# liuzuxin/FSRL

Hardware: NVIDIA H100
Metric: env-steps/sec (collect+update) SafetyCarCircle-v0 PPO-Lag (higher is better)
Workload: dtype f32

## Files before the change

### fsrl_b200/csrc/ppo_persist.cu

```cuda
#include "ppo_persist.cuh"
#include "arena.cuh"
#include "ppo_loss.cuh"
#include "wgmma.cuh"
#include <cstdlib>
#include <cmath>
#include <vector>

namespace fsrl {
namespace pp {

using namespace wg;

constexpr int WQ = 2;
constexpr int NEPI = 128 * WQ;
constexpr int TPB = NEPI + 32;
constexpr int C1 = 16 / WQ;
constexpr int C2 = 32 / WQ;
constexpr int RB = 64;
constexpr int MB = 256;
constexpr int KC = 32, NCH = 256 / KC;
constexpr int SLOT_BYTES = 32768, NSLOT = 4;
constexpr int A_CHUNK = 64 * KC * 4;
constexpr int ACC_LD = 68;
constexpr int OUTP = 8;
constexpr int H_ = 256;
constexpr int IMG = 65536;
enum { I_H1A_HI, I_H1A_LO, I_H1T_HI, I_H1T_LO, I_DZA_HI, I_DZA_LO, I_DZT_HI, I_DZT_LO, I_W2A_HI, I_W2A_LO, I_W2B_HI, I_W2B_LO, N_IMG };
constexpr int DB2P_OFF = N_IMG * IMG;
constexpr int DW3P_OFF = DB2P_OFF + 4 * H_;
constexpr int DB3P_OFF = DW3P_OFF + 4 * H_ * OUTP;
constexpr int DW1P_OFF = DB3P_OFF + 4 * 16;
constexpr int MAXD = 40;
constexpr int NET_WS = DW1P_OFF + 4 * WQ * (MAXD + 1) * H_;
constexpr int SUMSQ_FLOATS = 128;
constexpr int FLAG_LINE = 32;
constexpr int F_A = 0, F_C = 1, F_D1 = 2, F_PER_NET = 3;
constexpr int NSMAX = (MAXD + 1) * 32 + 32 + 32 * OUTP + 16;
constexpr int TILE_PK = (64 * 64 / NEPI + 2) / 3;
constexpr int TILE_FLOATS = TILE_PK * NEPI * 4;
constexpr int SLICE_PK = (NSMAX + 2) / 3;
constexpr int XG_PER_NET = 16 * TILE_FLOATS + 8 * SLICE_PK * 4;
constexpr int MAX_MB = 16384;
constexpr long long WAIT_CYCLES = 6000000000LL;

struct Args {
    fsrl_ppo_update_t u;
    int n_mb, slot0;
    long long adam_t0;
    float* ws;
    unsigned* flags;
    int* err;
    const float* adam_tab;
    long long* dbg;
    int dbg_step;
    unsigned dp_seq;
    int dp_direct;
};
constexpr int DBG_N = 48;
#define STAMP(i) do { if (P.dbg && t == P.dbg_step) P.dbg[(size_t)blockIdx.x * DBG_N + (i)] = clock64(); } while (0)

struct AdamS { float w1, b2, w2, rbc2s, eps, neg_step; };
__device__ __forceinline__ float adam_one(float p, float g, float& m, float& v, const AdamS& a) {
    m = m + a.w1 * (g - m);
    v = v * a.b2 + (a.w2 * g) * g;
    const float sq = v > 0.f ? v * rsqrtf(v) : 0.f;
    const float denom = fmaf(sq, a.rbc2s, a.eps);
    return p + __fdividef(a.neg_step * m, denom);
}

__device__ __forceinline__ void fail(int* err, int code) {
    *reinterpret_cast<volatile int*>(err) = code;
    __threadfence_system();
    asm volatile("trap;");
}
__device__ __forceinline__ uint32_t pk_hash(float x, float y, float z) {
    const uint32_t a = __float_as_uint(x), b = __float_as_uint(y), c = __float_as_uint(z);
    return a ^ __funnelshift_l(b, b, 11) ^ __funnelshift_l(c, c, 22);
}
__device__ __forceinline__ bool pk_ok(const float4& v, uint32_t tag) { return (__float_as_uint(v.w) ^ pk_hash(v.x, v.y, v.z)) == tag; }
__device__ __forceinline__ void st_packet(float* p, float x, float y, float z, uint32_t tag) {
    asm volatile("st.relaxed.sys.global.v4.f32 [%0], {%1,%2,%3,%4};" ::"l"(p), "f"(x), "f"(y), "f"(z), "f"(__uint_as_float(tag ^ pk_hash(x, y, z))) : "memory");
}
__device__ __forceinline__ float4 ld_packet(const float* p) {
    float4 v;
    asm volatile("ld.relaxed.sys.global.v4.f32 {%0,%1,%2,%3}, [%4];" : "=f"(v.x), "=f"(v.y), "=f"(v.z), "=f"(v.w) : "l"(p) : "memory");
    return v;
}

__device__ __noinline__ float3 dp_gather(const float* src, long long stride, int me, int world, uint32_t tag,
                                        float ox, float oy, float oz, int* err, int code) {
    const long long t0w = clock64();
    float ax = 0.f, ay = 0.f, az = 0.f;
    for (int r0 = 0; r0 < world; r0 += 4) {
        float4 v[4];
        bool ok;
        do {
            ok = true;
#pragma unroll
            for (int k = 0; k < 4; ++k)
                if (r0 + k < world && r0 + k != me) v[k] = ld_packet(src + (size_t)(r0 + k) * stride);
#pragma unroll
            for (int k = 0; k < 4; ++k)
                if (r0 + k < world && r0 + k != me) ok = ok && pk_ok(v[k], tag);
            if (!ok && clock64() - t0w > 4 * WAIT_CYCLES) fail(err, code);
        } while (!ok);
#pragma unroll
        for (int k = 0; k < 4; ++k) {
            if (r0 + k >= world) continue;
            if (r0 + k == me) { ax += ox; ay += oy; az += oz; }
            else { ax += v[k].x; ay += v[k].y; az += v[k].z; }
        }
    }
    return make_float3(ax, ay, az);
}
__device__ __noinline__ void dp_push_all(const float* const* xg, size_t off, int me, int world, float x, float y, float z, uint32_t tag) {
    for (int r = 0; r < world; ++r)
        if (r != me) st_packet(const_cast<float*>(xg[r]) + off, x, y, z, tag);
}

__device__ __forceinline__ uint32_t mapa_u32(uint32_t local_saddr, uint32_t rank) {
    uint32_t r;
    asm volatile("mapa.shared::cluster.u32 %0, %1, %2;" : "=r"(r) : "r"(local_saddr), "r"(rank));
    return r;
}
__device__ __forceinline__ void st_cluster4(uint32_t raddr, float4 v) {
    asm volatile("st.shared::cluster.v4.f32 [%0], {%1,%2,%3,%4};" ::"r"(raddr), "f"(v.x), "f"(v.y), "f"(v.z), "f"(v.w) : "memory");
}
__device__ __forceinline__ void st_async4(uint32_t raddr, float4 v, uint32_t rbar) {
    asm volatile("st.async.weak.shared::cluster.mbarrier::complete_tx::bytes.v4.f32 [%0], {%1,%2,%3,%4}, [%5];"
                 ::"r"(raddr), "f"(v.x), "f"(v.y), "f"(v.z), "f"(v.w), "r"(rbar) : "memory");
}
__device__ __forceinline__ bool mbar_wait_cluster(uint64_t* bar, uint32_t parity, long long timeout_cycles) {
    const long long t0 = clock64();
    while (true) {
        uint32_t ok;
        asm volatile(
            "{\n\t.reg .pred p;\n\t"
            "mbarrier.try_wait.parity.acquire.cluster.shared::cta.b64 p, [%1], %2;\n\t"
            "selp.u32 %0, 1, 0, p;\n\t}"
            : "=r"(ok) : "r"(smem_u32(bar)), "r"(parity) : "memory");
        if (ok) return true;
        if (clock64() - t0 > timeout_cycles) return false;
    }
}
__device__ __forceinline__ void cluster_sync_all() {
    asm volatile("barrier.cluster.arrive.release.aligned;\n\tbarrier.cluster.wait.acquire.aligned;" ::: "memory");
}

__device__ __forceinline__ bool elect_one() {
    uint32_t pred = 0;
    asm volatile(
        "{\n\t.reg .b32 rx;\n\t.reg .pred px;\n\t"
        "elect.sync rx|px, 0xffffffff;\n\t"
        "selp.u32 %0, 1, 0, px;\n\t}"
        : "=r"(pred));
    return pred != 0;
}
__device__ __forceinline__ void epi_bar() { asm volatile("bar.sync 1, %0;" ::"n"(NEPI) : "memory"); }
__device__ __forceinline__ void prefetch_l2(const void* p) { asm volatile("prefetch.global.L2 [%0];" ::"l"(p)); }

template <int NC>
__device__ __forceinline__ void acc_ld(const float* accs, int row, int col, float (&v)[NC]) {
#pragma unroll
    for (int q = 0; q < NC / 4; ++q) {
        const float4 x = *reinterpret_cast<const float4*>(accs + row * ACC_LD + col + 4 * q);
        v[4 * q] = x.x; v[4 * q + 1] = x.y; v[4 * q + 2] = x.z; v[4 * q + 3] = x.w;
    }
}
template <int NC>
__device__ __forceinline__ void acc_st(float* accs, int row, int col, const float (&v)[NC]) {
#pragma unroll
    for (int q = 0; q < NC / 4; ++q)
        *reinterpret_cast<float4*>(accs + row * ACC_LD + col + 4 * q) = make_float4(v[4 * q], v[4 * q + 1], v[4 * q + 2], v[4 * q + 3]);
}

template <int N>
__device__ __forceinline__ void gemm_phase(const unsigned char* ring, unsigned& qq, uint64_t* bar_full, uint32_t empty_r,
                                           float (&dm)[N / 2], float (&dc)[N / 2], int* err, int code, int lane) {
#pragma unroll
    for (int e = 0; e < N / 2; ++e) dm[e] = dc[e] = 0.f;
    const uint32_t ring_a = smem_u32(ring);
    constexpr uint32_t b_lbo = 16 * N, b_chunk = N * KC * 4;
    for (int j = 0; j < NCH; ++j, ++qq) {
        const int s = qq % NSLOT;
        if (!mbar_wait(&bar_full[s], (qq / NSLOT) & 1, WAIT_CYCLES)) fail(err, code);
        __syncwarp();
        wgmma_fence();
        const uint32_t base = ring_a + (uint32_t)s * SLOT_BYTES;
        const uint64_t ah0 = smem_desc(base, 1024, 128), al0 = smem_desc(base + A_CHUNK, 1024, 128);
        const uint64_t bh0 = smem_desc(base + 2 * A_CHUNK, b_lbo, 128), bl0 = smem_desc(base + 2 * A_CHUNK + b_chunk, b_lbo, 128);
#pragma unroll
        for (int ks = 0; ks < KC / 8; ++ks) {
            const uint64_t ah = ah0 + ks * (2048 / 16), al = al0 + ks * (2048 / 16);
            const uint64_t bh = bh0 + ks * (2 * b_lbo / 16), bl = bl0 + ks * (2 * b_lbo / 16);
            if constexpr (N == 32) {
                mma_m64n32k8_tf32(dc, al, bh);
                mma_m64n32k8_tf32(dc, ah, bl);
                mma_m64n32k8_tf32(dm, ah, bh);
            } else {
                mma_m64n64k8_tf32(dc, al, bh);
                mma_m64n64k8_tf32(dc, ah, bl);
                mma_m64n64k8_tf32(dm, ah, bh);
            }
        }
        wgmma_commit();
        if (j > 0) {
            wgmma_wait<1>();
            __syncwarp();
            if (lane < 8) mbar_arrive_cluster(empty_r + 8 * ((qq - 1) % NSLOT));
        }
    }
    wgmma_wait<0>();
    reg_fence(dm); reg_fence(dc);
    __syncwarp();
// ... 99 lines not shown
    float g[C2];
    acc_ld<C2>(accs, trow, cb2, g);
    const float inv_world = 1.0f / (float)d.world;
    const float* loc = d.xg[d.me];
#pragma unroll
    for (int q = 0; q < TILE_PK; ++q) {
        if (dp_owner(et, q, d.world) != d.me) continue;
        const float3 s3 = dp_gather(loc + off + (size_t)q * NEPI * 4, d.region, d.me, d.world, d.tag, g[3 * q],
                                    3 * q + 1 < C2 ? g[3 * q + 1] : 0.f, 3 * q + 2 < C2 ? g[3 * q + 2] : 0.f, d.err, 41);
        const float ax = s3.x * inv_world, ay = s3.y * inv_world, az = s3.z * inv_world;
        dp_push_all(d.xg, (size_t)FSRL_P2P_MAX_RANKS * d.region + off + (size_t)q * NEPI * 4, d.me, d.world, ax, ay, az, d.tag);
        g[3 * q] = ax;
        if (3 * q + 1 < C2) g[3 * q + 1] = ay;
        if (3 * q + 2 < C2) g[3 * q + 2] = az;
    }
    acc_st<C2>(accs, trow, cb2, g);
}
__device__ __noinline__ float dp_tile_finish(DpCtx d, size_t off, float* accs, int trow, int cb2, int et) {
    float g[C2];
    const long long t0w = clock64();
    if (d.direct) {
        float own[C2];
        acc_ld<C2>(accs, trow, cb2, own);
#pragma unroll
        for (int jq = 0; jq < C2; ++jq) g[jq] = 0.f;
        for (int r = 0; r < d.world; ++r) {
            if (r == d.me) {
#pragma unroll
                for (int jq = 0; jq < C2; ++jq) g[jq] += own[jq];
                continue;
            }
            const float* src = d.xg[d.me] + (size_t)r * d.region + off;
            float4 v[TILE_PK];
            bool ok;
            do {
                ok = true;
#pragma unroll
                for (int q = 0; q < TILE_PK; ++q) v[q] = ld_packet(src + (size_t)q * NEPI * 4);
#pragma unroll
                for (int q = 0; q < TILE_PK; ++q) ok = ok && pk_ok(v[q], d.tag);
                if (!ok && clock64() - t0w > 4 * WAIT_CYCLES) fail(d.err, 42);
            } while (!ok);
#pragma unroll
            for (int q = 0; q < TILE_PK; ++q) {
                g[3 * q] += v[q].x;
                if (3 * q + 1 < C2) g[3 * q + 1] += v[q].y;
                if (3 * q + 2 < C2) g[3 * q + 2] += v[q].z;
            }
        }
        const float inv_world = 1.0f / (float)d.world;
        float sq = 0.f;
#pragma unroll
        for (int jq = 0; jq < C2; ++jq) { g[jq] *= inv_world; sq = fmaf(g[jq], g[jq], sq); }
        acc_st<C2>(accs, trow, cb2, g);
        return sq;
    }
    const float* res = d.xg[d.me] + (size_t)FSRL_P2P_MAX_RANKS * d.region + off;
    acc_ld<C2>(accs, trow, cb2, g);
    float4 v[TILE_PK];
    bool ok;
    do {
        ok = true;
#pragma unroll
        for (int q = 0; q < TILE_PK; ++q)
            if (dp_owner(et, q, d.world) != d.me) v[q] = ld_packet(res + (size_t)q * NEPI * 4);
#pragma unroll
        for (int q = 0; q < TILE_PK; ++q)
            if (dp_owner(et, q, d.world) != d.me) ok = ok && pk_ok(v[q], d.tag);
        if (!ok && clock64() - t0w > 4 * WAIT_CYCLES) fail(d.err, 42);
    } while (!ok);
    float sq = 0.f;
#pragma unroll
    for (int q = 0; q < TILE_PK; ++q) {
        if (dp_owner(et, q, d.world) == d.me) continue;
        g[3 * q] = v[q].x;
        if (3 * q + 1 < C2) g[3 * q + 1] = v[q].y;
        if (3 * q + 2 < C2) g[3 * q + 2] = v[q].z;
    }
#pragma unroll
    for (int jq = 0; jq < C2; ++jq) sq = fmaf(g[jq], g[jq], sq);
    acc_st<C2>(accs, trow, cb2, g);
    return sq;
}
__device__ __noinline__ void dp_slices(DpCtx d, size_t off_s, float* sp_g, int n, int et, bool push) {
    const int n3 = (n + 2) / 3;
    const float inv_world = 1.0f / (float)d.world;
    if (push)
        for (int i = et; i < n3; i += NEPI)
            dp_push_all(d.xg, (size_t)d.me * d.region + off_s + 4 * (size_t)i, d.me, d.world,
                        sp_g[3 * i], 3 * i + 1 < n ? sp_g[3 * i + 1] : 0.f, 3 * i + 2 < n ? sp_g[3 * i + 2] : 0.f, d.tag);
    const float* loc = d.xg[d.me];
    for (int i = et; i < n3; i += NEPI) {
        const float3 s3 = dp_gather(loc + off_s + 4 * (size_t)i, d.region, d.me, d.world, d.tag, sp_g[3 * i],
                                    3 * i + 1 < n ? sp_g[3 * i + 1] : 0.f, 3 * i + 2 < n ? sp_g[3 * i + 2] : 0.f, d.err, 40);
        sp_g[3 * i] = s3.x * inv_world;
        if (3 * i + 1 < n) sp_g[3 * i + 1] = s3.y * inv_world;
        if (3 * i + 2 < n) sp_g[3 * i + 2] = s3.z * inv_world;
    }
}

template <bool DP>
__global__ void __launch_bounds__(TPB, 1) ppo_persist_kernel(const Args P) {
    extern __shared__ __align__(1024) unsigned char smem_raw[];
    __shared__ __align__(8) uint64_t bar_full[NSLOT], bar_empty[NSLOT], bar_b;
    __shared__ float s_red[4][320];
    __shared__ float s_misc[32];
    __shared__ AdamS s_adam;
    __shared__ const float* s_xg[2][FSRL_P2P_MAX_RANKS];
    const fsrl_ppo_update_t& u = P.u;
    const int tid = threadIdx.x, warp = tid >> 5, lane = tid & 31;
    const int net = blockIdx.x >> 5, c = blockIdx.x & 31, a = c >> 3, b = c & 7;
    const bool is_g2 = c < 16;
    const int ka = (c & 15) >> 2, q4 = c & 3;
    const int D = u.D, A = u.A, C = u.C, H = H_;
    const int out = (net == 0) ? A : 1;
    const int n_cta = 32 * u.n_nets;
    float* wsn = P.ws + (size_t)net * NET_WS;
    float* sumsq_g = P.ws + (size_t)u.n_nets * NET_WS;
    unsigned* fl_net = P.flags + (size_t)net * F_PER_NET * FLAG_LINE;
    unsigned* fl_d2 = P.flags + (size_t)u.n_nets * F_PER_NET * FLAG_LINE;
    unsigned char* ring = smem_raw;
    float* accs = reinterpret_cast<float*>(smem_raw + NSLOT * SLOT_BYTES);
    float* small = accs + 64 * ACC_LD;
    const SliceMap sm(D);
    float* sp_p = small;
    float* sp_m = small + sm.n;
    float* sp_v = small + 2 * sm.n;
    float* sp_g = small + 3 * sm.n;
    float* land = small + 4 * sm.n;

    if (tid == 0) {
        for (int i = 0; i < NSLOT; ++i) { mbar_init(&bar_full[i], 1); mbar_init(&bar_empty[i], 4 * 8); }
        mbar_init(&bar_b, 1);
        fence_mbar_init();
    }
    __syncthreads();
    if (DP && threadIdx.x < 2 * FSRL_P2P_MAX_RANKS) s_xg[threadIdx.x / FSRL_P2P_MAX_RANKS][threadIdx.x % FSRL_P2P_MAX_RANKS] = P.u.p2p_xg[threadIdx.x / FSRL_P2P_MAX_RANKS][threadIdx.x % FSRL_P2P_MAX_RANKS];
    if (DP) __syncthreads();
    cluster_sync_all();

    const long long pbase = u.net_off[net];
    const ArenaLayout L = arena_layout(D, H, out, 0);
    const long long o_w1 = pbase + L.w1, o_b1 = pbase + L.b1, o_w2 = pbase + L.w2, o_b2 = pbase + L.b2,
                    o_w3 = pbase + L.w3, o_b3 = pbase + L.b3, o_ls = pbase + L.extra;

    if (warp == NEPI / 32) {
        if (elect_one()) {
            unsigned qq = 0;
            for (int t = 0; t < P.n_mb; ++t) {
                if (!flag_wait_ge<true>(fl_net + F_A * FLAG_LINE, 32u * (t + 1), WAIT_CYCLES)) fail(P.err, 10);
                STAMP(12);
                fence_proxy_async();
#pragma unroll 1
                for (int j = 0; j < NCH; ++j, ++qq) {
                    const int s = qq % NSLOT;
                    if (!mbar_wait(&bar_empty[s], ((qq / NSLOT) & 1) ^ 1, WAIT_CYCLES)) fail(P.err, 11);
                    unsigned char* dst = ring + (size_t)s * SLOT_BYTES;
                    mbar_expect_tx(&bar_full[s], 3 * A_CHUNK);
                    const size_t ao = (size_t)a * 16384 + (size_t)j * 64 * KC, bo = (size_t)b * 8192 + (size_t)j * 32 * KC;
                    copy_operand(dst, wsn + (size_t)I_H1A_HI * IMG + ao, A_CHUNK, &bar_full[s], 8, b, 0xff);
                    copy_operand(dst + 2 * A_CHUNK, wsn + (size_t)I_W2A_HI * IMG + bo, A_CHUNK / 2, &bar_full[s], 1, 0, 0);
                }
                STAMP(13);
                if (!flag_wait_ge<true>(fl_net + F_C * FLAG_LINE, 32u * (t + 1), WAIT_CYCLES)) fail(P.err, 12);
                STAMP(14);
                fence_proxy_async();
                const int ia = is_g2 ? I_W2B_HI : I_DZT_HI, ib = is_g2 ? I_DZA_HI : I_H1T_HI;
                const int blk_a = is_g2 ? ka : q4, blk_b = is_g2 ? q4 : ka;
                const uint16_t m4 = (uint16_t)(0xfu << (b & 4)), m2 = (uint16_t)(0x11u << (b & 3));
#pragma unroll 1
                for (int j = 0; j < NCH; ++j, ++qq) {
                    const int s = qq % NSLOT;
                    if (!mbar_wait(&bar_empty[s], ((qq / NSLOT) & 1) ^ 1, WAIT_CYCLES)) fail(P.err, 13);
                    unsigned char* dst = ring + (size_t)s * SLOT_BYTES;
                    mbar_expect_tx(&bar_full[s], 4 * A_CHUNK);
                    const size_t ao = (size_t)blk_a * 16384 + (size_t)j * 64 * KC, bo = (size_t)blk_b * 16384 + (size_t)j * 64 * KC;
                    copy_operand(dst, wsn + (size_t)ia * IMG + ao, A_CHUNK, &bar_full[s], is_g2 ? 4 : 2, is_g2 ? b & 3 : b >> 2, is_g2 ? m4 : m2);
                    copy_operand(dst + 2 * A_CHUNK, wsn + (size_t)ib * IMG + bo, A_CHUNK, &bar_full[s], is_g2 ? 2 : 4, is_g2 ? b >> 2 : b & 3, is_g2 ? m2 : m4);
                }
            }
        }
    } else {
        const int et = tid;
        const int sp = warp & 3;
        const int wq = warp >> 2;
        const int r16 = lane & 15, half = lane >> 4;
        const int trow = 16 * sp + r16;
        const int cb1 = 16 * half + C1 * wq;
        const int cb2 = 32 * half + C2 * wq;
        unsigned qq = 0;
        const uint32_t empty_r = mapa_u32(smem_u32(bar_empty), lane < 8 ? lane : 0);
        float w2p[C2], w2m[C2], w2v[C2];
        const int world = DP ? u.world : 1;
        auto dp_ctx = [&](int t_) {
            DpCtx d;
            const unsigned long long id = (unsigned long long)(P.adam_t0 + t_ + 1);
            d.xg = s_xg[(int)(id & 1ULL)];
            d.region = (long long)u.n_nets * XG_PER_NET;
            d.me = u.p2p_rank; d.world = world;
            d.tag = (P.dp_seq << 16) | (uint32_t)((t_ + 1) & 0xffff);
            d.err = P.err;
            d.direct = P.dp_direct;
            return d;
        };

        for (int i = et; i < sm.n; i += NEPI) {
            long long src = -1;
            if (i < sm.b2) { const int d = i / 32, kk = i % 32; src = (d < D) ? o_w1 + (long long)d * H + 32 * b + kk : o_b1 + 32 * b + kk; }
            else if (i < sm.w3) src = o_b2 + 32 * b + (i - sm.b2);
            else if (i < sm.b3) { const int oo = (i - sm.w3) / OUTP, jj = (i - sm.w3) % OUTP; if (jj < out) src = o_w3 + (long long)(32 * b + oo) * out + jj; }
            else { const int jj = i - sm.b3; if (jj < out) src = o_b3 + jj; else if (net == 0 && jj >= 8 && jj < 8 + A) src = o_ls + (jj - 8); }
            sp_p[i] = src >= 0 ? u.theta[src] : 0.f;
            sp_m[i] = src >= 0 ? u.adam_m[src] : 0.f;
            sp_v[i] = src >= 0 ? u.adam_v[src] : 0.f;
            sp_g[i] = 0.f;
        }
// ... 209 lines not shown
#pragma unroll
                for (int q = 0; q < C1 / 4; ++q) {
#pragma unroll
                    for (int e = 0; e < 4; ++e) tf32_split(dz[4 * q + e], hi[4 * q + e], lo[4 * q + e]);
                    const size_t plane = (size_t)(8 * b + (cb1 >> 2) + q) * 256;
                    *reinterpret_cast<float4*>(a_hi + plane) = make_float4(hi[4 * q], hi[4 * q + 1], hi[4 * q + 2], hi[4 * q + 3]);
                    *reinterpret_cast<float4*>(a_hi + IMG + plane) = make_float4(lo[4 * q], lo[4 * q + 1], lo[4 * q + 2], lo[4 * q + 3]);
                }
                store_transposed<C1, 32>(scratch, hi, lo, trow, cb1, et, wsn + (size_t)I_DZT_HI * IMG + (size_t)(b >> 1) * 16384, 64 * a, 32 * (b & 1));
            }
            if (et == 0) STAMP(27);
            {
                float* row = &s_red[sp][0];
#pragma unroll
                for (int j = 0; j < C1; ++j) {
                    const float sdz = half_sum(dz[j]);
                    if (r16 == 0) row[cb1 + j] = sdz;
                }
#pragma unroll
                for (int jj = 0; jj < OUTP; ++jj) {
                    if (jj < nfeed) {
#pragma unroll
                        for (int j = 0; j < C1; ++j) {
                            const float sv = half_sum(h2[j] * dd[jj]);
                            if (r16 == 0) row[32 + 32 * jj + cb1 + j] = sv;
                        }
                    }
                }
                if (b == 0 && wq == 0) {
#pragma unroll
                    for (int j = 0; j < 16; ++j) {
                        const float sv = half_sum(dd[j]);
                        if (lane == 0) row[288 + j] = sv;
                    }
                    const float sa = half_sum(st_a), sb = half_sum(st_b), sc = half_sum(st_c), sdv = half_sum(st_d);
                    if (lane == 0) { row[304] = sa; row[305] = sb; row[306] = sc; row[307] = sdv; }
                }
            }
            epi_bar();
            if (et == 0) STAMP(28);
            for (int i = et; i < 32 + 32 * nfeed; i += NEPI) {
                const float tot = ((s_red[0][i] + s_red[1][i]) + s_red[2][i]) + s_red[3][i];
                if (i < 32) wsn[DB2P_OFF + a * H + 32 * b + i] = tot;
                else wsn[DW3P_OFF + ((size_t)a * H + 32 * b + ((i - 32) & 31)) * OUTP + ((i - 32) >> 5)] = tot;
            }
            if (b == 0) {
                if (et < 20) {
                    const int i = 288 + et;
                    const float tot = ((s_red[0][i] + s_red[1][i]) + s_red[2][i]) + s_red[3][i];
                    if (et < 16) wsn[DB3P_OFF + a * 16 + et] = tot;
                    else {
                        float* stat = u.stats + (size_t)slot * FSRL_PPO_STATS;
                        if (net == 0) { if (et == 16) atomicAdd(stat + ST_ACTOR_REW, tot); if (et == 17) atomicAdd(stat + ST_ACTOR_SAFETY, tot); if (et == 18) atomicAdd(stat + ST_KL, tot); }
                        else if (et == 19) atomicAdd(stat + ST_VF0 + (net - 1), tot);
                    }
                }
                if (net == 0 && a == 0 && et == 20) u.stats[(size_t)slot * FSRL_PPO_STATS + ST_ENTROPY] = ppo_entropy(sp_p + sm.b3 + 8, A);
            }
            fence_proxy_async_smem();
            epi_bar();
            if (et == 0) { STAMP(5); flag_add_release(fl_net + F_C * FLAG_LINE); }

            unsigned mbits = 0;
            if (is_g2) {
                const int k = 64 * ka + trow;
                const float* msk = wsn + (size_t)I_H1A_HI * IMG + (size_t)q4 * 16384 + (size_t)(k >> 2) * 256 + (k & 3);
                float mreg[C2];
#pragma unroll
                for (int jq = 0; jq < C2; ++jq) mreg[jq] = __ldcg(msk + (size_t)(cb2 + jq) * 4);
                float xr[(64 * MAXD + NEPI - 1) / NEPI];
                const int nx = (64 * D + NEPI - 1) / NEPI;
                const float* xb = u.obs + (row0 + 64 * q4) * D;
#pragma unroll
                for (int q = 0; q < (64 * MAXD + NEPI - 1) / NEPI; ++q)
                    xr[q] = (q < nx && et + q * NEPI < 64 * D) ? __ldg(xb + et + q * NEPI) : 0.f;
#pragma unroll
                for (int jq = 0; jq < C2; ++jq) mbits |= (mreg[jq] > 0.f ? 1u : 0u) << jq;
#pragma unroll
                for (int q = 0; q < (64 * MAXD + NEPI - 1) / NEPI; ++q) {
                    const int e = et + q * NEPI;
                    if (q < nx && e < 64 * D) { const int r = e / D; land[e + (r >> 5)] = xr[q]; }
                }
            }
            {
                float dm[32], dc[32];
                if (wq == 0) gemm_phase<64>(ring, qq, bar_full, empty_r, dm, dc, P.err, 32, lane);
                else qq += NCH;
                stage_acc<64>(accs, dm, dc, wq, sp, lane);
            }
            if (et == 0) STAMP(6);
            float sq = 0.f;
            if (is_g2) {
                float v[C2];
                acc_ld<C2>(accs, trow, cb2, v);
                const int k = 64 * ka + trow;
#pragma unroll
                for (int jq = 0; jq < C2; ++jq) v[jq] = ((mbits >> jq) & 1u) ? v[jq] : 0.f;
                epi_bar();
                if (et == 0) STAMP(22);
                const float* xh = land + (size_t)cb2 * D + half;
                float* dst = wsn + DW1P_OFF + (size_t)(WQ * q4 + wq) * (MAXD + 1) * H + k;
                for (int d = 0; d < D; ++d) {
                    float sacc = 0.f;
#pragma unroll
                    for (int jq = 0; jq < C2; ++jq) sacc = fmaf(xh[jq * D + d], v[jq], sacc);
                    sacc += __shfl_xor_sync(0xffffffffu, sacc, 16);
                    if (half == 0) dst[(size_t)d * H] = sacc;
                }
                float sb1 = 0.f;
#pragma unroll
                for (int jq = 0; jq < C2; ++jq) sb1 += v[jq];
                sb1 += __shfl_xor_sync(0xffffffffu, sb1, 16);
                if (half == 0) dst[(size_t)D * H] = sb1;
                if (et == 0) STAMP(23);
                epi_bar();
                if (et == 0) flag_add_release(fl_net + F_D1 * FLAG_LINE);
            } else {
                float g[C2];
                acc_ld<C2>(accs, trow, cb2, g);
                if (DP) {
                    dp_tile_send(dp_ctx(t), (size_t)(net * 16 + (c - 16)) * TILE_FLOATS + (size_t)et * 4, accs, trow, cb2, et);
                    if (et == 0) STAMP(32);
                } else {
#pragma unroll
                    for (int jq = 0; jq < C2; ++jq) sq = fmaf(g[jq], g[jq], sq);
                }
            }
            auto reduce_slices = [&](int lo, int hi) {
                for (int i0 = lo + et; i0 < hi; i0 += 4 * NEPI) {
                    float pv[4][4 * WQ];
                    bool real[4];
                    int np[4];
#pragma unroll
                    for (int e = 0; e < 4; ++e) {
                        const int i = i0 + e * NEPI;
                        const float* src = wsn;
                        size_t stride = 0;
                        real[e] = false;
                        np[e] = 4;
                        if (i < hi) {
                            if (i < sm.b2) { src = wsn + DW1P_OFF + (size_t)(i / 32) * H + 32 * b + (i % 32); stride = (size_t)(MAXD + 1) * H; real[e] = true; np[e] = 4 * WQ; }
                            else if (i < sm.w3) { src = wsn + DB2P_OFF + 32 * b + (i - sm.b2); stride = H; real[e] = true; }
                            else if (i < sm.b3) {
                                const int oo = (i - sm.w3) / OUTP, jj = (i - sm.w3) % OUTP;
                                real[e] = jj < out;
                                src = wsn + DW3P_OFF + ((size_t)32 * b + oo) * OUTP + jj; stride = (size_t)H * OUTP;
                            } else {
                                const int jj = i - sm.b3;
                                real[e] = (jj < out) || (net == 0 && jj >= 8 && jj < 8 + A);
                                src = wsn + DB3P_OFF + jj; stride = 16;
                            }
                        }
#pragma unroll
                        for (int q = 0; q < 4 * WQ; ++q) pv[e][q] = (real[e] && q < np[e]) ? __ldcg(src + q * stride) : 0.f;
                    }
#pragma unroll
                    for (int e = 0; e < 4; ++e) {
                        const int i = i0 + e * NEPI;
                        if (i < hi) {
                            float gsum = 0.f;
#pragma unroll
                            for (int q = 0; q < 4 * WQ; ++q) gsum += pv[e][q];
                            sp_g[i] = gsum;
                        }
                    }
                }
            };
            reduce_slices(sm.b2, sm.n);
            if (et == 0) { STAMP(7); if (!flag_wait_ge(fl_net + F_D1 * FLAG_LINE, 16u * (t + 1), WAIT_CYCLES)) fail(P.err, 33); STAMP(8); }
            epi_bar();
            reduce_slices(0, sm.b2);
            if (DP) {
                const DpCtx d = dp_ctx(t);
                const size_t off_t = (size_t)(net * 16 + (c - 16)) * TILE_FLOATS + (size_t)et * 4;
                epi_bar();
                if (!is_g2 && !d.direct) { dp_tile_reduce(d, off_t, accs, trow, cb2, et); if (et == 0) STAMP(33); }
                dp_slices(d, (size_t)u.n_nets * 16 * TILE_FLOATS + (size_t)(net * 8 + b) * SLICE_PK * 4, sp_g, sm.n, et, a == 0);
                __syncwarp();
                if (et == 0) STAMP(38);
                if (!is_g2) { sq += dp_tile_finish(d, off_t, accs, trow, cb2, et); if (et == 0) STAMP(41); }
                epi_bar();
            }
            if (a == 0) {
                for (int i = et; i < sm.n; i += NEPI) {
                    bool real = true;
                    if (i >= sm.w3 && i < sm.b3) real = ((i - sm.w3) % OUTP) < out;
                    else if (i >= sm.b3) { const int jj = i - sm.b3; real = (jj < out) || (net == 0 && jj >= 8 && jj < 8 + A); }
                    if (real && (i < sm.b3 || b == 0)) sq = fmaf(sp_g[i], sp_g[i], sq);
                }
            }
            sq = warp_sum(sq);
            if (lane == 0) s_misc[warp] = sq;
            epi_bar();
            if (et == 0) {
                float tot = 0.f;
#pragma unroll
                for (int w2 = 0; w2 < NEPI / 32; ++w2) tot += s_misc[w2];
                sumsq_g[blockIdx.x] = tot;
                STAMP(9);
                flag_add_release(fl_d2);
                if (!flag_wait_ge(fl_d2, (unsigned)n_cta * (t + 1), WAIT_CYCLES)) fail(P.err, 34);
                STAMP(10);
            }
            epi_bar();
            float nq[4];
#pragma unroll
            for (int q = 0; q < 4; ++q) nq[q] = (lane + 32 * q < n_cta) ? __ldcg(sumsq_g + lane + 32 * q) : 0.f;
            float nsq = ((nq[0] + nq[1]) + nq[2]) + nq[3];
            nsq = warp_sum(nsq);
            float gscale = 1.0f;
            if (u.max_grad_norm > 0.f) gscale = fminf(u.max_grad_norm / (sqrtf(nsq) + 1e-6f), 1.0f);
            if (blockIdx.x == 0 && et == 0) u.stats[(size_t)slot * FSRL_PPO_STATS + ST_GRADNORM] = sqrtf(nsq);
            const AdamS ad = s_adam;
            if (et == 0) STAMP(24);
            for (int i = et; i < sm.n; i += NEPI) {
                float m = sp_m[i], v = sp_v[i];
                sp_p[i] = adam_one(sp_p[i], sp_g[i] * gscale, m, v, ad);
                sp_m[i] = m; sp_v[i] = v;
            }
            if (et == 0) STAMP(25);
            if (!is_g2) {
                float g[C2];
                acc_ld<C2>(accs, trow, cb2, g);
#pragma unroll
                for (int j = 0; j < C2; ++j) w2p[j] = adam_one(w2p[j], g[j] * gscale, w2m[j], w2v[j], ad);
            }
            epi_bar();
            if (et == 0) STAMP(11);
        }

        if (a == 0) {
            for (int i = et; i < sm.n; i += NEPI) {
                long long dst = -1;
                if (i < sm.b2) { const int d = i / 32, kk = i % 32; dst = (d < D) ? o_w1 + (long long)d * H + 32 * b + kk : o_b1 + 32 * b + kk; }
                else if (i < sm.w3) dst = o_b2 + 32 * b + (i - sm.b2);
                else if (i < sm.b3) { const int oo = (i - sm.w3) / OUTP, jj = (i - sm.w3) % OUTP; if (jj < out) dst = o_w3 + (long long)(32 * b + oo) * out + jj; }
                else if (b == 0) { const int jj = i - sm.b3; if (jj < out) dst = o_b3 + jj; else if (net == 0 && jj >= 8 && jj < 8 + A) dst = o_ls + (jj - 8); }
                if (dst >= 0) { u.theta[dst] = sp_p[i]; u.adam_m[dst] = sp_m[i]; u.adam_v[dst] = sp_v[i]; }
            }
        }
        if (!is_g2) {
            const int o = 64 * q4 + trow;
#pragma unroll
            for (int j = 0; j < C2; ++j) {
                const long long idx = o_w2 + (long long)(64 * ka + cb2 + j) * H + o;
                u.theta[idx] = w2p[j]; u.adam_m[idx] = w2m[j]; u.adam_v[idx] = w2v[j];
            }
        }
    }
    __syncthreads();
    cluster_sync_all();
}

static size_t smem_bytes(int D) {
    return (size_t)NSLOT * SLOT_BYTES + sizeof(float) * 64 * ACC_LD + 4 * sizeof(float) * SliceMap(D).n +
           sizeof(float) * 8 * 64 * OUTP;
}

static cudaLaunchConfig_t cluster_launch(int n_nets, size_t smem, cudaStream_t s, cudaLaunchAttribute* at) {
    at->id = cudaLaunchAttributeClusterDimension;
    at->val.clusterDim.x = 8; at->val.clusterDim.y = 1; at->val.clusterDim.z = 1;
    cudaLaunchConfig_t cfg = {};
    cfg.gridDim = dim3(32 * n_nets); cfg.blockDim = dim3(TPB); cfg.dynamicSmemBytes = smem; cfg.stream = s;
    cfg.attrs = at; cfg.numAttrs = 1;
    return cfg;
}

struct Instance {
    void (*kern)(const Args);
    int max_clusters;
};
static const Instance& instance(bool dp) {
    static Instance inst[2] = {};
    Instance& in = inst[dp];
    if (!in.kern) {
        in.kern = dp ? ppo_persist_kernel<true> : ppo_persist_kernel<false>;
        cudaLaunchAttribute at;
        const cudaLaunchConfig_t cfg = cluster_launch(1, smem_bytes(MAXD), nullptr, &at);
        if (cudaFuncSetAttribute(in.kern, cudaFuncAttributeMaxDynamicSharedMemorySize, (int)cfg.dynamicSmemBytes) != cudaSuccess ||
            cudaOccupancyMaxActiveClusters(&in.max_clusters, in.kern, &cfg) != cudaSuccess) {
            cudaGetLastError();
            in.max_clusters = 0;
        }
    }
    return in;
}

}

size_t ppo_persist_ws_floats(int n_nets, int D, int H) {
    (void)D; (void)H;
    return (size_t)n_nets * pp::NET_WS + pp::SUMSQ_FLOATS + (size_t)(n_nets * pp::F_PER_NET + 1) * pp::FLAG_LINE + 32 +
           2 * (size_t)pp::MAX_MB + 2 * (size_t)32 * n_nets * pp::DBG_N;
}

size_t ppo_persist_p2p_floats(int n_nets) { return (size_t)(FSRL_P2P_MAX_RANKS + 1) * n_nets * pp::XG_PER_NET + 64; }

bool ppo_persist_supported(const fsrl_ppo_update_t& u, long long n_total, int batch_size) {
    if (u.H != 256 || batch_size != pp::MB || n_total % pp::MB != 0 || n_total < pp::MB || n_total / pp::MB > pp::MAX_MB) return false;
    if (u.world > 1 && !(u.p2p_on && u.world <= FSRL_P2P_MAX_RANKS && (size_t)u.p2p_stride >= ppo_persist_p2p_floats(u.n_nets))) return false;
    if (u.D < 1 || u.D > pp::MAXD || u.A > 8 || u.n_nets < 1 || u.n_nets > 3) return false;
    if (u.persist_ws == nullptr || (size_t)u.persist_ws_floats < ppo_persist_ws_floats(u.n_nets, u.D, u.H)) return false;
    if (32 * u.n_nets > sm_count()) return false;
    return pp::instance(u.world > 1).max_clusters >= 4 * u.n_nets;
}

int ppo_persist_run(const fsrl_ppo_update_t& ug, int n_mb, int stats_slot0, long long adam_t0, cudaStream_t s) {
    pp::Args a;
    a.u = ug;
    a.n_mb = n_mb; a.slot0 = stats_slot0; a.adam_t0 = adam_t0;
    a.ws = ug.persist_ws;
    const size_t fl_off = (size_t)ug.n_nets * pp::NET_WS + pp::SUMSQ_FLOATS;
    a.flags = reinterpret_cast<unsigned*>(ug.persist_ws + fl_off);
    const size_t n_flag_words = (size_t)(ug.n_nets * pp::F_PER_NET + 1) * pp::FLAG_LINE;
    a.err = reinterpret_cast<int*>(a.flags + n_flag_words);
    FSRL_CUDA(cudaMemsetAsync(a.flags, 0, (n_flag_words + 32) * sizeof(unsigned), s));
    float* tab_dev = reinterpret_cast<float*>(a.err + 32);
    static std::vector<float> tab;
    tab.resize(2 * (size_t)n_mb);
    for (int t = 0; t < n_mb; ++t) {
        const double tt = (double)(adam_t0 + t + 1);
        const double bc1 = 1.0 - pow(ug.beta1, tt), bc2 = 1.0 - pow(ug.beta2, tt);
        tab[2 * t] = (float)(1.0 / sqrt(bc2));
        tab[2 * t + 1] = (float)(-(ug.lr / bc1));
    }
    FSRL_CUDA(cudaMemcpyAsync(tab_dev, tab.data(), tab.size() * sizeof(float), cudaMemcpyHostToDevice, s));
    a.adam_tab = tab_dev;
    static unsigned dp_seq = 0;
    if (ug.world > 1) dp_seq = (dp_seq % 65535u) + 1u;
    a.dp_seq = dp_seq;
    a.dp_direct = ug.world <= 2;
    if (const char* e = getenv("FSRL_PPO_DP_DIRECT")) a.dp_direct = atoi(e) != 0;
    a.dbg = nullptr; a.dbg_step = -1;
    if (const char* e = getenv("FSRL_PPO_PERSIST_DBG")) {
        a.dbg = reinterpret_cast<long long*>(tab_dev + 2 * (size_t)pp::MAX_MB);
        a.dbg_step = atoi(e);
    }
    cudaLaunchAttribute at;
    const cudaLaunchConfig_t cfg = pp::cluster_launch(ug.n_nets, pp::smem_bytes(ug.D), s, &at);
    FSRL_CUDA(cudaLaunchKernelEx(&cfg, pp::instance(ug.world > 1).kern, a));
    ++g_launches;
    return FSRL_OK;
}

}
```

Baseline: 2.611 million.

## Reduce W1 gradient slices through cluster DSMEM with mbarrier signalling

Per-CTA W1 gradient partials now stay in shared memory (the ring buffer) and are summed by designated reducer CTAs, which read them over distributed shared memory after a cluster mbarrier arrive. Before, every CTA wrote them to global workspace and waited on a global flag. The small b2/w3/b3 slice reduction moves earlier, onto the second warpgroup of the reducer CTAs, so it overlaps with the GEMM phase. Only reducer CTAs and g1 CTAs now take part in the global sum-of-squares barrier. The other CTAs read reduced slices back from a global slice buffer, which adds an extra global round trip and tighter coupling to the cluster layout.

```diff
diff --git a/fsrl_b200/csrc/ppo_persist.cu b/fsrl_b200/csrc/ppo_persist.cu
--- a/fsrl_b200/csrc/ppo_persist.cu
+++ b/fsrl_b200/csrc/ppo_persist.cu
@@ -29,13 +29,13 @@
 constexpr int DB2P_OFF = N_IMG * IMG;
 constexpr int DW3P_OFF = DB2P_OFF + 4 * H_;
 constexpr int DB3P_OFF = DW3P_OFF + 4 * H_ * OUTP;
-constexpr int DW1P_OFF = DB3P_OFF + 4 * 16;
 constexpr int MAXD = 40;
-constexpr int NET_WS = DW1P_OFF + 4 * WQ * (MAXD + 1) * H_;
+constexpr int NSMAX = (MAXD + 1) * 32 + 32 + 32 * OUTP + 16;
+constexpr int SLICE_OFF = DB3P_OFF + 4 * 16;
+constexpr int NET_WS = SLICE_OFF + 8 * NSMAX;
 constexpr int SUMSQ_FLOATS = 128;
 constexpr int FLAG_LINE = 32;
-constexpr int F_A = 0, F_C = 1, F_D1 = 2, F_PER_NET = 3;
-constexpr int NSMAX = (MAXD + 1) * 32 + 32 + 32 * OUTP + 16;
+constexpr int F_A = 0, F_C = 1, F_PER_NET = 2;
 constexpr int TILE_PK = (64 * 64 / NEPI + 2) / 3;
 constexpr int TILE_FLOATS = TILE_PK * NEPI * 4;
 constexpr int SLICE_PK = (NSMAX + 2) / 3;
@@ -130,6 +130,14 @@
     asm volatile("st.async.weak.shared::cluster.mbarrier::complete_tx::bytes.v4.f32 [%0], {%1,%2,%3,%4}, [%5];"
                  ::"r"(raddr), "f"(v.x), "f"(v.y), "f"(v.z), "f"(v.w), "r"(rbar) : "memory");
 }
+__device__ __forceinline__ float ld_cluster(uint32_t raddr) {
+    float v;
+    asm volatile("ld.shared::cluster.f32 %0, [%1];" : "=f"(v) : "r"(raddr) : "memory");
+    return v;
+}
+__device__ __forceinline__ void mbar_arrive_release_cluster(uint32_t raddr) {
+    asm volatile("mbarrier.arrive.release.cluster.shared::cluster.b64 _, [%0];" ::"r"(raddr) : "memory");
+}
 __device__ __forceinline__ bool mbar_wait_cluster(uint64_t* bar, uint32_t parity, long long timeout_cycles) {
     const long long t0 = clock64();
     while (true) {
@@ -395,13 +403,12 @@
     acc_st<C2>(accs, trow, cb2, g);
     return sq;
 }
-__device__ __noinline__ void dp_slices(DpCtx d, size_t off_s, float* sp_g, int n, int et, bool push) {
+__device__ __noinline__ void dp_slices(DpCtx d, size_t off_s, float* sp_g, int n, int et) {
     const int n3 = (n + 2) / 3;
     const float inv_world = 1.0f / (float)d.world;
-    if (push)
-        for (int i = et; i < n3; i += NEPI)
-            dp_push_all(d.xg, (size_t)d.me * d.region + off_s + 4 * (size_t)i, d.me, d.world,
-                        sp_g[3 * i], 3 * i + 1 < n ? sp_g[3 * i + 1] : 0.f, 3 * i + 2 < n ? sp_g[3 * i + 2] : 0.f, d.tag);
+    for (int i = et; i < n3; i += NEPI)
+        dp_push_all(d.xg, (size_t)d.me * d.region + off_s + 4 * (size_t)i, d.me, d.world,
+                    sp_g[3 * i], 3 * i + 1 < n ? sp_g[3 * i + 1] : 0.f, 3 * i + 2 < n ? sp_g[3 * i + 2] : 0.f, d.tag);
     const float* loc = d.xg[d.me];
     for (int i = et; i < n3; i += NEPI) {
         const float3 s3 = dp_gather(loc + off_s + 4 * (size_t)i, d.region, d.me, d.world, d.tag, sp_g[3 * i],
@@ -412,10 +419,20 @@
     }
 }
 
+__device__ __forceinline__ bool red_cta() { return ((blockIdx.x >> 3) & 3) == ((blockIdx.x & 7) >> 2); }
+
+__device__ __noinline__ float dp_tail(DpCtx d, size_t off_t, size_t off_s, float* accs, float* sp_g, int n, int trow, int cb2,
+                                      int et, bool tile, bool slice) {
+    if (tile && !d.direct) dp_tile_reduce(d, off_t, accs, trow, cb2, et);
+    if (slice) dp_slices(d, off_s, sp_g, n, et);
+    __syncwarp();
+    return tile ? dp_tile_finish(d, off_t, accs, trow, cb2, et) : 0.f;
+}
+
 template <bool DP>
 __global__ void __launch_bounds__(TPB, 1) ppo_persist_kernel(const Args P) {
     extern __shared__ __align__(1024) unsigned char smem_raw[];
-    __shared__ __align__(8) uint64_t bar_full[NSLOT], bar_empty[NSLOT], bar_b;
+    __shared__ __align__(8) uint64_t bar_full[NSLOT], bar_empty[NSLOT], bar_b, bar_w1;
     __shared__ float s_red[4][320];
     __shared__ float s_misc[32];
     __shared__ AdamS s_adam;
@@ -425,6 +442,7 @@
     const int net = blockIdx.x >> 5, c = blockIdx.x & 31, a = c >> 3, b = c & 7;
     const bool is_g2 = c < 16;
     const int ka = (c & 15) >> 2, q4 = c & 3;
+
     const int D = u.D, A = u.A, C = u.C, H = H_;
     const int out = (net == 0) ? A : 1;
     const int n_cta = 32 * u.n_nets;
@@ -445,6 +463,7 @@
     if (tid == 0) {
         for (int i = 0; i < NSLOT; ++i) { mbar_init(&bar_full[i], 1); mbar_init(&bar_empty[i], 4 * 8); }
         mbar_init(&bar_b, 1);
+        mbar_init(&bar_w1, 4);
         fence_mbar_init();
     }
     __syncthreads();
@@ -820,6 +839,49 @@
                     if (q < nx && e < 64 * D) { const int r = e / D; land[e + (r >> 5)] = xr[q]; }
                 }
             }
+            if (red_cta() && wq == 1) {
+                const int tw = et - 128;
+                if (tw == 0) {
+                    if (!flag_wait_ge(fl_net + F_C * FLAG_LINE, 32u * (t + 1), WAIT_CYCLES)) fail(P.err, 35);
+                    STAMP(15);
+                }
+                asm volatile("bar.sync 6, 128;" ::: "memory");
+                for (int i0 = sm.b2 + tw; i0 < sm.n; i0 += 4 * 128) {
+                    float pv[4][4];
+#pragma unroll
+                    for (int e = 0; e < 4; ++e) {
+                        const int i = i0 + e * 128;
+                        const float* src = wsn;
+                        size_t stride = 0;
+                        bool real = false;
+                        if (i < sm.n) {
+                            if (i < sm.w3) { src = wsn + DB2P_OFF + 32 * b + (i - sm.b2); stride = H; real = true; }
+                            else if (i < sm.b3) {
+                                const int oo = (i - sm.w3) / OUTP, jj = (i - sm.w3) % OUTP;
+                                real = jj < out;
+                                src = wsn + DW3P_OFF + ((size_t)32 * b + oo) * OUTP + jj; stride = (size_t)H * OUTP;
+                            } else {
+                                const int jj = i - sm.b3;
+                                real = (jj < out) || (net == 0 && jj >= 8 && jj < 8 + A);
+                                src = wsn + DB3P_OFF + jj; stride = 16;
+                            }
+                        }
+#pragma unroll
+                        for (int q = 0; q < 4; ++q) pv[e][q] = real ? __ldcg(src + q * stride) : 0.f;
+                    }
+#pragma unroll
+                    for (int e = 0; e < 4; ++e) {
+                        const int i = i0 + e * 128;
+                        if (i < sm.n) {
+                            float gsum = 0.f;
+#pragma unroll
+                            for (int q = 0; q < 4; ++q) gsum += pv[e][q];
+                            sp_g[i] = gsum;
+                        }
+                    }
+                }
+                if (tw == 0) STAMP(16);
+            }
             {
                 float dm[32], dc[32];
                 if (wq == 0) gemm_phase<64>(ring, qq, bar_full, empty_r, dm, dc, P.err, 32, lane);
@@ -831,28 +893,30 @@
             if (is_g2) {
                 float v[C2];
                 acc_ld<C2>(accs, trow, cb2, v);
-                const int k = 64 * ka + trow;
 #pragma unroll
                 for (int jq = 0; jq < C2; ++jq) v[jq] = ((mbits >> jq) & 1u) ? v[jq] : 0.f;
                 epi_bar();
                 if (et == 0) STAMP(22);
                 const float* xh = land + (size_t)cb2 * D + half;
-                float* dst = wsn + DW1P_OFF + (size_t)(WQ * q4 + wq) * (MAXD + 1) * H + k;
+                float* dst = reinterpret_cast<float*>(ring) + (size_t)wq * (D + 1) * 64 + trow;
                 for (int d = 0; d < D; ++d) {
                     float sacc = 0.f;
 #pragma unroll
                     for (int jq = 0; jq < C2; ++jq) sacc = fmaf(xh[jq * D + d], v[jq], sacc);
                     sacc += __shfl_xor_sync(0xffffffffu, sacc, 16);
-                    if (half == 0) dst[(size_t)d * H] = sacc;
+                    if (half == 0) dst[d * 64] = sacc;
                 }
                 float sb1 = 0.f;
 #pragma unroll
                 for (int jq = 0; jq < C2; ++jq) sb1 += v[jq];
                 sb1 += __shfl_xor_sync(0xffffffffu, sb1, 16);
-                if (half == 0) dst[(size_t)D * H] = sb1;
+                if (half == 0) dst[D * 64] = sb1;
                 if (et == 0) STAMP(23);
                 epi_bar();
-                if (et == 0) flag_add_release(fl_net + F_D1 * FLAG_LINE);
+                if (et == 0) {
+                    mbar_arrive_release_cluster(mapa_u32(smem_u32(&bar_w1), 2 * ka));
+                    mbar_arrive_release_cluster(mapa_u32(smem_u32(&bar_w1), 2 * ka + 1));
+                }
             } else {
                 float g[C2];
                 acc_ld<C2>(accs, trow, cb2, g);
@@ -864,38 +928,30 @@
                     for (int jq = 0; jq < C2; ++jq) sq = fmaf(g[jq], g[jq], sq);
                 }
             }
-            auto reduce_slices = [&](int lo, int hi) {
-                for (int i0 = lo + et; i0 < hi; i0 += 4 * NEPI) {
-                    float pv[4][4 * WQ];
-                    bool real[4];
-                    int np[4];
-#pragma unroll
-                    for (int e = 0; e < 4; ++e) {
+            if (et == 0) STAMP(7);
+            if (red_cta()) {
+                if (!mbar_wait_cluster(&bar_w1, t & 1, WAIT_CYCLES)) fail(P.err, 33);
+                if (et == 0) STAMP(8);
+                const uint32_t ring_s = smem_u32(ring);
+                const int kb = 32 * (b & 1);
+                for (int i0 = et; i0 < sm.b2; i0 += 2 * NEPI) {
+                    float pv[2][4 * WQ];
+#pragma unroll
+                    for (int e = 0; e < 2; ++e) {
                         const int i = i0 + e * NEPI;
-                        const float* src = wsn;
-                        size_t stride = 0;
-                        real[e] = false;
-                        np[e] = 4;
-                        if (i < hi) {
-                            if (i < sm.b2) { src = wsn + DW1P_OFF + (size_t)(i / 32) * H + 32 * b + (i % 32); stride = (size_t)(MAXD + 1) * H; real[e] = true; np[e] = 4 * WQ; }
-                            else if (i < sm.w3) { src = wsn + DB2P_OFF + 32 * b + (i - sm.b2); stride = H; real[e] = true; }
-                            else if (i < sm.b3) {
-                                const int oo = (i - sm.w3) / OUTP, jj = (i - sm.w3) % OUTP;
-                                real[e] = jj < out;
-                                src = wsn + DW3P_OFF + ((size_t)32 * b + oo) * OUTP + jj; stride = (size_t)H * OUTP;
-                            } else {
-                                const int jj = i - sm.b3;
-                                real[e] = (jj < out) || (net == 0 && jj >= 8 && jj < 8 + A);
-                                src = wsn + DB3P_OFF + jj; stride = 16;
-                            }
+                        const uint32_t off = 4u * (uint32_t)((i / 32) * 64 + kb + (i % 32));
+#pragma unroll
+                        for (int rb = 0; rb < 4; ++rb) {
+                            const uint32_t src = mapa_u32(ring_s + off, (uint32_t)((4 * (b >> 1) + rb) & 7));
+#pragma unroll
+                            for (int w = 0; w < WQ; ++w)
+                                pv[e][WQ * rb + w] = i < sm.b2 ? ld_cluster(src + 4u * (uint32_t)(w * (D + 1) * 64)) : 0.f;
                         }
-#pragma unroll
-                        for (int q = 0; q < 4 * WQ; ++q) pv[e][q] = (real[e] && q < np[e]) ? __ldcg(src + q * stride) : 0.f;
                     }
 #pragma unroll
-                    for (int e = 0; e < 4; ++e) {
+                    for (int e = 0; e < 2; ++e) {
                         const int i = i0 + e * NEPI;
-                        if (i < hi) {
+                        if (i < sm.b2) {
                             float gsum = 0.f;
 #pragma unroll
                             for (int q = 0; q < 4 * WQ; ++q) gsum += pv[e][q];
@@ -903,47 +959,49 @@
                         }
                     }
                 }
-            };
-            reduce_slices(sm.b2, sm.n);
-            if (et == 0) { STAMP(7); if (!flag_wait_ge(fl_net + F_D1 * FLAG_LINE, 16u * (t + 1), WAIT_CYCLES)) fail(P.err, 33); STAMP(8); }
-            epi_bar();
-            reduce_slices(0, sm.b2);
+                epi_bar();
+                if (et == 0) STAMP(17);
+            }
             if (DP) {
                 const DpCtx d = dp_ctx(t);
                 const size_t off_t = (size_t)(net * 16 + (c - 16)) * TILE_FLOATS + (size_t)et * 4;
+                sq += dp_tail(d, off_t, (size_t)u.n_nets * 16 * TILE_FLOATS + (size_t)(net * 8 + b) * SLICE_PK * 4, accs, sp_g, sm.n,
+                              trow, cb2, et, !is_g2, red_cta());
+                if (et == 0) STAMP(41);
                 epi_bar();
-                if (!is_g2 && !d.direct) { dp_tile_reduce(d, off_t, accs, trow, cb2, et); if (et == 0) STAMP(33); }
-                dp_slices(d, (size_t)u.n_nets * 16 * TILE_FLOATS + (size_t)(net * 8 + b) * SLICE_PK * 4, sp_g, sm.n, et, a == 0);
-                __syncwarp();
-                if (et == 0) STAMP(38);
-                if (!is_g2) { sq += dp_tile_finish(d, off_t, accs, trow, cb2, et); if (et == 0) STAMP(41); }
-                epi_bar();
-            }
-            if (a == 0) {
+            }
+            if (red_cta()) {
                 for (int i = et; i < sm.n; i += NEPI) {
                     bool real = true;
                     if (i >= sm.w3 && i < sm.b3) real = ((i - sm.w3) % OUTP) < out;
                     else if (i >= sm.b3) { const int jj = i - sm.b3; real = (jj < out) || (net == 0 && jj >= 8 && jj < 8 + A); }
                     if (real && (i < sm.b3 || b == 0)) sq = fmaf(sp_g[i], sp_g[i], sq);
-                }
-            }
-            sq = warp_sum(sq);
-            if (lane == 0) s_misc[warp] = sq;
-            epi_bar();
+                    wsn[SLICE_OFF + (size_t)b * NSMAX + i] = sp_g[i];
+                }
+            }
+            if (red_cta() || !is_g2) {
+                sq = warp_sum(sq);
+                if (lane == 0) s_misc[warp] = sq;
+                epi_bar();
+                if (et == 0) {
+                    float tot = 0.f;
+#pragma unroll
+                    for (int w2 = 0; w2 < NEPI / 32; ++w2) tot += s_misc[w2];
+                    sumsq_g[blockIdx.x - (red_cta() ? 8 * a : 0)] = tot;
+                    STAMP(9);
+                    flag_add_release(fl_d2);
+                }
+            }
             if (et == 0) {
-                float tot = 0.f;
-#pragma unroll
-                for (int w2 = 0; w2 < NEPI / 32; ++w2) tot += s_misc[w2];
-                sumsq_g[blockIdx.x] = tot;
-                STAMP(9);
-                flag_add_release(fl_d2);
-                if (!flag_wait_ge(fl_d2, (unsigned)n_cta * (t + 1), WAIT_CYCLES)) fail(P.err, 34);
+                if (!flag_wait_ge(fl_d2, 24u * (unsigned)u.n_nets * (t + 1), WAIT_CYCLES)) fail(P.err, 34);
                 STAMP(10);
             }
             epi_bar();
             float nq[4];
 #pragma unroll
             for (int q = 0; q < 4; ++q) nq[q] = (lane + 32 * q < n_cta) ? __ldcg(sumsq_g + lane + 32 * q) : 0.f;
+            if (!DP && !red_cta())
+                for (int i = et; i < sm.n; i += NEPI) sp_g[i] = __ldcg(wsn + SLICE_OFF + (size_t)b * NSMAX + i);
             float nsq = ((nq[0] + nq[1]) + nq[2]) + nq[3];
             nsq = warp_sum(nsq);
             float gscale = 1.0f;
@@ -953,7 +1011,8 @@
             if (et == 0) STAMP(24);
             for (int i = et; i < sm.n; i += NEPI) {
                 float m = sp_m[i], v = sp_v[i];
-                sp_p[i] = adam_one(sp_p[i], sp_g[i] * gscale, m, v, ad);
+                const float g = (DP && !red_cta()) ? __ldcg(wsn + SLICE_OFF + (size_t)b * NSMAX + i) : sp_g[i];
+                sp_p[i] = adam_one(sp_p[i], g * gscale, m, v, ad);
                 sp_m[i] = m; sp_v[i] = v;
             }
             if (et == 0) STAMP(25);
@@ -1052,7 +1111,7 @@
     a.flags = reinterpret_cast<unsigned*>(ug.persist_ws + fl_off);
     const size_t n_flag_words = (size_t)(ug.n_nets * pp::F_PER_NET + 1) * pp::FLAG_LINE;
     a.err = reinterpret_cast<int*>(a.flags + n_flag_words);
-    FSRL_CUDA(cudaMemsetAsync(a.flags, 0, (n_flag_words + 32) * sizeof(unsigned), s));
+    FSRL_CUDA(cudaMemsetAsync(ug.persist_ws + fl_off - pp::SUMSQ_FLOATS, 0, (pp::SUMSQ_FLOATS + n_flag_words + 32) * sizeof(float), s));
     float* tab_dev = reinterpret_cast<float*>(a.err + 32);
     static std::vector<float> tab;
     tab.resize(2 * (size_t)n_mb);
```

After: 2.746 million, median of 6. 1.05x the previous value.
